# xingbpshen/nested-diffusion

Hardware: AMD Instinct MI355X
Metric: denoising-steps*images/sec (K=5,T=100,224^2) (higher is better)
Workload: dtype f32

## Files before the change

nested_diffusion_amd/csrc/nd_sampler.hip:

```cpp
#include "nd_common.hpp"
#include "nd_step.hpp"
#include "nd_cond_gemm.hpp"
#include "nd_b9.hpp"
#include "nd_persist.hpp"
#include "nd_rng.hpp"
#include "../../include/nested_diffusion.h"

#include <map>
#include <string>
#include <tuple>
#include <vector>
#include <cstdio>
#include <cstdarg>
#include <cstring>
#include <cstdlib>

static thread_local std::string g_err;
extern "C" const char* nd_last_error(void) { return g_err.c_str(); }
#ifdef ND_WG_TIMING
int nd_debug_set_wg_times_m0(void*); int nd_debug_set_wg_times_m1(void*); int nd_debug_set_wg_times_m2(void*);
extern "C" int nd_debug_set_wg_times(void* dev_ptr) {
    return (nd_debug_set_wg_times_m0(dev_ptr) | nd_debug_set_wg_times_m1(dev_ptr) | nd_debug_set_wg_times_m2(dev_ptr)) ? -1 : 0;
}
#endif
// ... 87 lines not shown
            zz[c] = ND_GC(io.noise)[z * io.noise_ms + ((size_t)i_step * M + m) * C + c];
        }
    }
    if (mode == ND_HEAD_UPDATE) {
        al = ND_GC(io.alphas)[t_prev]; s_t = ND_GC(io.omabs)[t_prev]; s_tm1 = ND_GC(io.omabs)[t_prev - 1];
#pragma unroll
        for (int c = 0; c < C; ++c) yo[c] = yold[c];
        nd_reduce_eps<256, C>(mb.epart, NT, m, red, eps);
    }
#pragma unroll
    for (int c = 0; c < C; ++c) {
        if (mode == ND_HEAD_INIT) yv[c] = zz[c] + ym[c];
        else if (mode == ND_HEAD_UPDATE) yv[c] = nd_posterior(yo[c], ym[c], eps[c] + ND_GC(mb.lin4_b)[c], zz[c], al, s_t, s_tm1);
        else yv[c] = ND_GC(io.y_in)[z * io.yin_ms + (size_t)m * C + c];
        if (tid == 0 && blockIdx.x == 0) {
            ynew[c] = yv[c];
            if (io.seq_out && mode != ND_HEAD_GIVEN) ND_GW(io.seq_out)[z * io.seq_ms + ((size_t)i_step * M + m) * C + c] = yv[c];
        }
    }
    if (!live) return;
    float4 h;
    h.x = nd_head_element<C>(w1[0], yv, yh, a.x, cc.x, xe.x);
    h.y = nd_head_element<C>(w1[1], yv, yh, a.y, cc.y, xe.y);
    h.z = nd_head_element<C>(w1[2], yv, yh, a.z, cc.z, xe.z);
    h.w = nd_head_element<C>(w1[3], yv, yh, a.w, cc.w, xe.w);
    if (mb.h16 == 2)
        nd_b9_store4(reinterpret_cast<bf16x8*>(mb.h1), F >> 5, m, n, h.x, h.y, h.z, h.w);
    else if (mb.h16)
        *(__attribute__((address_space(1))) f16x4*)(reinterpret_cast<_Float16*>(mb.h1) + nd_pkh(m, n, F >> 5)) =
            f16x4{(_Float16)h.x, (_Float16)h.y, (_Float16)h.z, (_Float16)h.w};
    else
        *(__attribute__((address_space(1))) f32x4*)(mb.h1 + nd_pk(m, n, nchF)) = f32x4{h.x, h.y, h.z, h.w};
}

#ifndef ND_HEAD_ROWS_COLS
#define ND_HEAD_ROWS_COLS 512
#endif
template <int C>
__global__ __launch_bounds__(256) void k_step_head_rows(MemberInline mi, const MemberDev* __restrict__ members, StepIO io, int mode,
                                                        int i_step, int t_prev, int t, int B, int M, int maxM, int F, int NT, int T) {
    typedef const __attribute__((address_space(4))) char* nd_cbytes;
    const MemberDev mb = nd_ldc<MemberDev>((members ? (nd_cbytes)(uintptr_t)members : (nd_cbytes)__builtin_amdgcn_kernarg_segment_ptr()) +
                                           (size_t)blockIdx.z * sizeof(MemberDev));
    const int z = blockIdx.z, tid = threadIdx.x, m0 = blockIdx.y * 16;
    constexpr int C2 = 2 * C;
    __shared__ float ys[16][C], yhs[16][C];
    {
        const int r = tid >> 4, j = tid & 15, m = min(m0 + r, M - 1), b = m % B;
        const int par_new = i_step & 1;
        nd_gf ynew = ND_GW(mb.ybuf + ((size_t)par_new * maxM + m) * C);
        nd_gcf yold = ND_GC(mb.ybuf + ((size_t)(par_new ^ 1) * maxM + m) * C);
        float yv[C], yh[C], ym[C], zz[C], yo[C], eps[C];
        float al = 0.f, s_t = 0.f, s_tm1 = 0.f;
#pragma unroll
        for (int c = 0; c < C; ++c) {
            yh[c] = ND_GC(io.yhat)[z * io.yhat_ms + (size_t)b * C + c];
            eps[c] = 0.f; ym[c] = 0.f; zz[c] = 0.f; yo[c] = 0.f;
        }
        if (mode != ND_HEAD_GIVEN) {
#pragma unroll
            for (int c = 0; c < C; ++c) {
                ym[c] = ND_GC(io.ymean)[z * io.ymean_ms + (size_t)b * C + c];
                zz[c] = ND_GC(io.noise)[z * io.noise_ms + ((size_t)i_step * M + m) * C + c];
            }
        }
        if (mode == ND_HEAD_UPDATE) {
            al = ND_GC(io.alphas)[t_prev]; s_t = ND_GC(io.omabs)[t_prev]; s_tm1 = ND_GC(io.omabs)[t_prev - 1];
#pragma unroll
            for (int c = 0; c < C; ++c) {
                yo[c] = yold[c];
                nd_gcf row = ND_GC(mb.epart + ((size_t)m * C + c) * NT);
                float q[4];
#pragma unroll
                for (int k = 0; k < 4; ++k) {
                    const int tl = j + 16 * k;
                    const float v = row[min(tl, NT - 1)];
                    q[k] = tl < NT ? 0.f + v : 0.f;
                }
                float s = (q[0] + q[2]) + (q[1] + q[3]);
#pragma unroll
                for (int off = 8; off > 0; off >>= 1) s += __shfl_down(s, off, 16);
                float tot = 0.f;
                tot += s;
                tot += 0.f; tot += 0.f; tot += 0.f;
                eps[c] = __shfl(tot, 0, 16);
            }
        }
#pragma unroll
        for (int c = 0; c < C; ++c) {
            if (mode == ND_HEAD_INIT) yv[c] = zz[c] + ym[c];
            else if (mode == ND_HEAD_UPDATE) yv[c] = nd_posterior(yo[c], ym[c], eps[c] + ND_GC(mb.lin4_b)[c], zz[c], al, s_t, s_tm1);
            else yv[c] = ND_GC(io.y_in)[z * io.yin_ms + (size_t)m * C + c];
            if (j == 0) {
                ys[r][c] = yv[c]; yhs[r][c] = yh[c];
                if (blockIdx.x == 0 && m0 + r < M) {
                    ynew[c] = yv[c];
                    if (io.seq_out && mode != ND_HEAD_GIVEN) ND_GW(io.seq_out)[z * io.seq_ms + ((size_t)i_step * M + m) * C + c] = yv[c];
                }
            }
        }
    }
    __syncthreads();
    const int lane = tid & 63, wave = tid >> 6, r = lane & 15, kq = lane >> 4;
    const int m = m0 + r, b = min(m, M - 1) % B, nkb = F >> 5, nchF = F >> 4;
    float yv[C], yh[C];
#pragma unroll
    for (int c = 0; c < C; ++c) { yv[c] = ys[r][c]; yh[c] = yhs[r][c]; }
    bf16x8* img = reinterpret_cast<bf16x8*>(mb.h1);
#pragma unroll
    for (int it = 0; it < ND_HEAD_ROWS_COLS / 128; ++it) {
        const int kb = blockIdx.x * (ND_HEAD_ROWS_COLS / 32) + wave * (ND_HEAD_ROWS_COLS / 128) + it;
        if (kb >= nkb) break;
        const int n = kb * 32 + kq * 8;
        const float4 a0 = nd_ld16<false>(mb.A1 + (size_t)t * F + n), a1 = nd_ld16<false>(mb.A1 + (size_t)t * F + n + 4);
        const float4 c0 = nd_ld16<false>(mb.C1 + (size_t)t * F + n), c1 = nd_ld16<false>(mb.C1 + (size_t)t * F + n + 4);
        const float4 x0 = nd_ld16<false>(mb.xe + nd_pk(b, n, nchF)), x1 = nd_ld16<false>(mb.xe + nd_pk(b, n + 4, nchF));
        const float av[8] = {a0.x, a0.y, a0.z, a0.w, a1.x, a1.y, a1.z, a1.w};
        const float cv[8] = {c0.x, c0.y, c0.z, c0.w, c1.x, c1.y, c1.z, c1.w};
        const float xv[8] = {x0.x, x0.y, x0.z, x0.w, x1.x, x1.y, x1.z, x1.w};
        nd_gcf wrow = ND_GC(mb.lin1_w + (size_t)n * C2);
        float w1[8][C2];
#pragma unroll
        for (int jj = 0; jj < 8; ++jj)
#pragma unroll
            for (int q = 0; q < C2; ++q) w1[jj][q] = wrow[jj * C2 + q];
        bf16x8 p1, p2, p3;
#pragma unroll
        for (int jj = 0; jj < 8; ++jj) {
            const float hv = nd_head_element<C>(w1[jj], yv, yh, av[jj], cv[jj], xv[jj]);
            __bf16 e1, e2, e3;
            nd_b9_split(hv, e1, e2, e3);
            p1[jj] = e1; p2[jj] = e2; p3[jj] = e3;
        }
        if (m < M) {
            __attribute__((address_space(1))) bf16x8* q = (__attribute__((address_space(1))) bf16x8*)(img + ((size_t)(m0 >> 4) * nkb + kb) * B9_BLOCK_UNITS + lane);
            q[0] = p1; q[64] = p2; q[128] = p3;
        }
    }
}

static void* head_rows_fn(int C) {
    switch (C) {
        case 1: return (void*)k_step_head_rows<1>;
        case 2: return (void*)k_step_head_rows<2>;
        case 3: return (void*)k_step_head_rows<3>;
        case 4: return (void*)k_step_head_rows<4>;
        case 5: return (void*)k_step_head_rows<5>;
        case 6: return (void*)k_step_head_rows<6>;
        case 7: return (void*)k_step_head_rows<7>;
        default: return (void*)k_step_head_rows<8>;
    }
}

static void* head_fn(int C) {
    switch (C) {
        case 1: return (void*)k_step_head<1>;
        case 2: return (void*)k_step_head<2>;
        case 3: return (void*)k_step_head<3>;
        case 4: return (void*)k_step_head<4>;
        case 5: return (void*)k_step_head<5>;
        case 6: return (void*)k_step_head<6>;
        case 7: return (void*)k_step_head<7>;
        default: return (void*)k_step_head<8>;
    }
}

template <int C>
__global__ __launch_bounds__(64) void k_step_final(MemberInline mi, const MemberDev* __restrict__ members, StepIO io, int eps_only, int par_cur,
                                                   int B, int M, int maxM, int NT, int T, float* eps_out, size_t eps_ms) {
    typedef const __attribute__((address_space(4))) char* nd_cbytes;
    const MemberDev mb = nd_ldc<MemberDev>((members ? (nd_cbytes)(uintptr_t)members : (nd_cbytes)__builtin_amdgcn_kernarg_segment_ptr()) +
                                           (size_t)blockIdx.z * sizeof(MemberDev));
    const int z = blockIdx.z, m = blockIdx.x, b = m % B;
    __shared__ float red[C];
    float epsv[C];
    nd_reduce_eps<64, C>(mb.epart, NT, m, red, epsv);
#pragma unroll
    for (int c = 0; c < C; ++c) {
        const float eps = epsv[c] + mb.lin4_b[c];
        if (threadIdx.x == 0) {
            if (eps_only == 1) {
                eps_out[z * eps_ms + (size_t)m * C + c] = eps;
            } else if (eps_only >= 2) {
                const float y = io.y_in[(size_t)m * C + c];
                const float ymean = io.ymean[(size_t)b * C + c];
                const int t = par_cur;
                eps_out[(size_t)m * C + c] = eps_only == 2
                    ? nd_posterior(y, ymean, eps, io.noise[(size_t)m * C + c], io.alphas[t], io.omabs[t], io.omabs[t - 1])
                    : nd_y0_reparam(y, ymean, eps, io.omabs[0]);
            } else {
                const float y = mb.ybuf[((size_t)par_cur * maxM + m) * C + c];
                const float ymean = io.ymean[z * io.ymean_ms + (size_t)b * C + c];
                const float y0 = nd_y0_reparam(y, ymean, eps, io.omabs[0]);
                io.y0_out[z * io.y0_ms + (size_t)m * C + c] = y0;
                if (io.seq_out) io.seq_out[z * io.seq_ms + ((size_t)T * M + m) * C + c] = y0;
            }
        }
    }
}

static void* final_fn(int C) {
    switch (C) {
        case 1: return (void*)k_step_final<1>;
        case 2: return (void*)k_step_final<2>;
        case 3: return (void*)k_step_final<3>;
        case 4: return (void*)k_step_final<4>;
        case 5: return (void*)k_step_final<5>;
        case 6: return (void*)k_step_final<6>;
        case 7: return (void*)k_step_final<7>;
        default: return (void*)k_step_final<8>;
    }
}

__global__ void k_fold_bn(float* scale, float* shift, const float* lin_b, const float* bn_w, const float* bn_b,
                          const float* bn_mean, const float* bn_var, int N) {
    const int n = blockIdx.x * blockDim.x + threadIdx.x;
    if (n >= N) return;
    const double s = (double)bn_w[n] / sqrt((double)bn_var[n] + 1e-5);
    const double o = (double)bn_b[n] - (double)bn_mean[n] * s;
    scale[n] = (float)s;
    shift[n] = (float)(s * (double)lin_b[n] + o);
}
__global__ void k_fold_steps(float* A, float* Cc, const float* emb, const float* lin_b, const float* bn_w, const float* bn_b,
                             const float* bn_mean, const float* bn_var, int T, int N) {
    const size_t i = (size_t)blockIdx.x * blockDim.x + threadIdx.x;
    if (i >= (size_t)T * N) return;
    const int n = (int)(i % N);
    const double s = (double)bn_w[n] / sqrt((double)bn_var[n] + 1e-5);
    const double o = (double)bn_b[n] - (double)bn_mean[n] * s;
    const double g = (double)emb[i];
    A[i] = (float)(s * g);
    Cc[i] = (float)(s * g * (double)lin_b[n] + o);
}

#define ND_KEEP_BYTES 208.0e6
enum { L_ENC0 = 0, L_ENC1 = 1, L_ENC2 = 2, L_LIN2 = 3, L_LIN3 = 4, L_LIN2S = 5, L_LIN3S = 6, L_COUNT = 7 };

struct MemberHost {
    bool loaded = false;
    float *sc0, *sh0, *sc1, *sh1, *sc2, *sh2;
    float *A[3], *Cc[3];
    float *w_enc0, *w_enc3, *w_enc6, *w_lin2, *w_lin3;
    float *w_lin1, *w_lin4, *b_lin4;
    float *e0, *e1, *xe, *ybuf, *h1, *h2, *epart, *splitk;
    void *w_lin2s = nullptr, *w_lin3s = nullptr, *h1s = nullptr, *h2s = nullptr;
    bool h_split = false;
};

struct GraphKey {
    int m0, nm, B, mc, T;
    const void *yhat, *ymean, *noise, *y0, *seq;
    bool operator<(const GraphKey& o) const {
        return std::tie(m0, nm, B, mc, T, yhat, ymean, noise, y0, seq) <
               std::tie(o.m0, o.nm, o.B, o.mc, o.T, o.yhat, o.ymean, o.noise, o.y0, o.seq);
    }
};

int nd_guiding_prediction_first(nd_cond c, const float* images, float* logits_out, float* yhat_out, int B, int n_used, void* stream);
unsigned long long nd_cond_serial(nd_cond c);

struct BatchKey {
    unsigned long long cond;
    const void *images, *noise, *samples, *prob, *vote, *probs, *yhat;
    int B, mc, T;
    unsigned temp_bits;
    bool profiling;
    bool operator<(const BatchKey& o) const {
        return std::tie(cond, images, noise, samples, prob, vote, probs, yhat, B, mc, T, temp_bits, profiling) <
               std::tie(o.cond, o.images, o.noise, o.samples, o.prob, o.vote, o.probs, o.yhat, o.B, o.mc, o.T, o.temp_bits, o.profiling);
    }
};

struct nd_handle_s {
    nd_config cfg{};
    char* ws = nullptr;
    size_t ws_bytes = 0;
    std::vector<MemberHost> members;
    MemberDev* members_dev = nullptr;
    SkinnyDesc* descs_dev = nullptr;
    std::vector<SkinnyDesc> descs_host;
    std::vector<MemberDev> members_host;
    SkinnyDesc* spk_dev = nullptr;
    SplitKEpiDesc* spke_dev = nullptr;
    float *alphas = nullptr, *omabs = nullptr;
    float* xpack = nullptr;
    float* tile_ws = nullptr;
    bool b9 = false;
    unsigned long long* rng_state = nullptr;
    unsigned* input_seq = nullptr;
    unsigned* input_flag = nullptr;
    unsigned* persist_bar = nullptr;
    int persist_mode = 0;
    int persist_skew_ticks = 0;
    bool persist_last = false;
    float* noise_ws = nullptr;
    float* logits_ws = nullptr;
    int sched_T = 0;
    int NT = 0, S0 = 0;
    bool enc_splitk = false;
    int half = 0;
    std::map<GraphKey, hipGraphExec_t> graphs;
    std::map<BatchKey, hipGraphExec_t> batch_graphs;
    hipStream_t capture_stream = nullptr;
    int encoded_B = -1;
    bool profiling = false;
    std::vector<hipEvent_t> probe_events;
    int probe_steps = 0;
    int probe_nodes = 0;
};

static inline size_t al256(size_t x) { return (x + 255) & ~(size_t)255; }

struct Carver {
    char* base; size_t off = 0;
    template <typename T> T* take(size_t count) {
        T* p = base ? reinterpret_cast<T*>(base + off) : nullptr;
        off = al256(off + count * sizeof(T));
// ... 283 lines not shown
    return encode_impl(h, m0, nm, x_dev, B, stream, false);
}

static int encode_impl(nd_handle h, int m0, int nm, const float* x_dev, int B, void* stream, bool signal_inputs) {
    int rc = check_range(h, m0, nm);
    if (rc != ND_OK) return rc;
    if (!x_dev) return nd_set_err(ND_ERR_ARG, "x_dev is NULL");
    if (B < 1 || B > h->cfg.max_batch) return nd_set_err(ND_ERR_ARG, "B=%d outside [1,%d]", B, h->cfg.max_batch);
    hipStream_t st = (hipStream_t)stream;
    const nd_config& c = h->cfg;
    const int K = c.n_members, H = c.hidden_dim, F = c.feature_dim, D = c.data_dim;
    launch_pack(x_dev, h->xpack, B, D, h->half, st);
    if (signal_inputs && h->input_flag)
        hipLaunchKernelGGL(k_inputs_consumed, dim3(1), dim3(1), 0, st, h->input_seq, h->input_flag);
    if (h->enc_splitk) {
        const SkinnyLaunch L = nd_skinny_launch<2>(D, H, B, nm, h->half);
        HIP_CHECK(nd_launch_skinny(L, SkinnyDesc{}, h->spk_dev + m0, nm, B, 0, st));
        const size_t q = (size_t)(((B + 15) / 16) * 16) * H / 4;
        hipLaunchKernelGGL(k_splitk_epilogue, dim3((unsigned)((q + 255) / 256), 1, nm), dim3(256), 0, st, SplitKEpiDesc{},
                           (const SplitKEpiDesc*)(h->spke_dev + m0), B, L.S);
    } else {
        HIP_CHECK(launch_skinny<0>(h->descs_dev + (size_t)L_ENC0 * K + m0, D, H, B, 0, nm, h->half, st));
    }
    HIP_CHECK(launch_skinny<0>(h->descs_dev + (size_t)L_ENC1 * K + m0, H, H, B, 0, nm, h->half, st));
    HIP_CHECK(launch_skinny<0>(h->descs_dev + (size_t)L_ENC2 * K + m0, H, F, B, 0, nm, h->half, st));
    HIP_CHECK(hipGetLastError());
    h->encoded_B = B;
    return ND_OK;
}

extern "C" int nd_member_buffer(nd_handle h, int k, int which, float* dst_dev, int rows, void* stream) {
    if (!h || !dst_dev) return nd_set_err(ND_ERR_ARG, "bad argument");
    if (k < 0 || k >= h->cfg.n_members) return nd_set_err(ND_ERR_ARG, "member out of range");
    if (which < 0 || which > 4) return nd_set_err(ND_ERR_ARG, "which=%d unknown", which);
    if (rows < 1 || rows > h->cfg.max_rows) return nd_set_err(ND_ERR_ARG, "rows out of range");
    const bool enc = which == 0 || which >= 3;
    if (enc && rows > h->cfg.max_batch) return nd_set_err(ND_ERR_ARG, "%s holds at most max_batch rows", which == 0 ? "xe" : which == 3 ? "e0" : "e1");
    if (!h->ws) return nd_set_err(ND_ERR_STATE, "workspace not bound");
    MemberHost& m = h->members[k];
    const float* src = which == 0 ? m.xe : which == 1 ? m.h1 : which == 2 ? m.h2 : which == 3 ? m.e0 : m.e1;
    const int W = which >= 3 ? h->cfg.hidden_dim : h->cfg.feature_dim;
    if (!enc && m.h_split) return nd_join_rows(which == 1 ? m.h1s : m.h2s, dst_dev, rows, W, stream);
    const size_t n4 = (size_t)((rows + 15) / 16) * 16 * W / 4;
    if (h->half && which != 0)
        hipLaunchKernelGGL(k_unpack_rows_h, dim3((unsigned)((n4 / 2 + 255) / 256)), dim3(256), 0, (hipStream_t)stream,
                           reinterpret_cast<const _Float16*>(src), dst_dev, rows, W);
    else
        hipLaunchKernelGGL(k_unpack_rows, dim3((unsigned)((n4 + 255) / 256)), dim3(256), 0, (hipStream_t)stream, src, dst_dev, rows, W);
    HIP_CHECK(hipGetLastError());
    return ND_OK;
}

extern "C" long long nd_resident_weight_bytes(nd_handle h, int block) {
    if (!h || block < 0 || block > 1 || h->descs_host.empty()) return -1;
    const int K = h->cfg.n_members, F = h->cfg.feature_dim;
    long long n = 0;
    for (int k = 0; k < K; ++k)
        if (h->members[k].loaded && h->descs_host[(size_t)(block ? L_LIN3 : L_LIN2) * K + k].keep) n += (long long)F * F * (h->half ? 2 : 4);
    return n;
}

extern "C" int nd_set_profiling(nd_handle h, int enable) {
    if (!h) return nd_set_err(ND_ERR_ARG, "handle is NULL");
    if (h->profiling != (enable != 0)) drop_graphs(h);
    h->profiling = enable != 0;
    return ND_OK;
}

extern "C" int nd_set_loop_form(nd_handle h, int mode, float skew_us) {
    if (!h) return nd_set_err(ND_ERR_ARG, "handle is NULL");
    if (mode != 0 && mode != 1) return nd_set_err(ND_ERR_ARG, "mode must be 0 (per-step kernels) or 1 (one launch per loop)");
    if (skew_us > 1e6f) return nd_set_err(ND_ERR_ARG, "skew_us out of range");
    h->persist_mode = mode;
    if (skew_us >= 0.f) h->persist_skew_ticks = (int)(skew_us * 100.0f);
    drop_graphs(h);
    return ND_OK;
}

extern "C" int nd_loop_form(nd_handle h) { return h && h->persist_last ? 1 : 0; }

extern "C" int nd_persist_status(nd_handle h, int reset) {
    if (!h || !h->ws) return nd_set_err(ND_ERR_STATE, "workspace not bound");
    HIP_CHECK(hipDeviceSynchronize());
    unsigned flag = 0;
    HIP_CHECK(hipMemcpy(&flag, h->persist_bar + ND_PERSIST_ERR_WORD, sizeof flag, hipMemcpyDeviceToHost));
    if (reset && flag) HIP_CHECK(hipMemset(h->persist_bar, 0, ND_PERSIST_BAR_WORDS * sizeof(unsigned)));
    return flag ? 1 : 0;
}

static int count_event_record_nodes(hipGraph_t g) {
    size_t n = 0;
    if (hipGraphGetNodes(g, nullptr, &n) != hipSuccess) return -1;
    std::vector<hipGraphNode_t> nodes(n);
    if (n && hipGraphGetNodes(g, nodes.data(), &n) != hipSuccess) return -1;
    int cnt = 0;
    for (size_t i = 0; i < n; ++i) {
        hipGraphNodeType ty;
        if (hipGraphNodeGetType(nodes[i], &ty) != hipSuccess) return -1;
        if (ty == hipGraphNodeTypeEventRecord) ++cnt;
    }
    return cnt;
}

extern "C" int nd_profile_probe_nodes(nd_handle h) {
    if (!h) return nd_set_err(ND_ERR_ARG, "handle is NULL");
    return h->probe_nodes;
}

extern "C" int nd_profile_read(nd_handle h, float* out_us, int* n_samples) {
    if (!h || !out_us || !n_samples) return nd_set_err(ND_ERR_ARG, "NULL argument");
    double acc[3] = {0, 0, 0};
    const int n = h->probe_steps;
    for (int s = 0; s < n; ++s)
        for (int k = 0; k < 3; ++k) {
            float ms = 0.f;
            HIP_CHECK(hipEventElapsedTime(&ms, h->probe_events[4 * s + k], h->probe_events[4 * s + k + 1]));
            acc[k] += ms * 1000.0;
        }
    out_us[0] = n ? (float)(acc[0] / n) : 0.f;
    out_us[1] = n ? (float)(acc[1] / n) : 0.f;
    out_us[2] = n ? (float)(acc[2] / n) : 0.f;
    const float head = out_us[2] - out_us[1];
    out_us[3] = n ? (out_us[0] - head > 0.f ? out_us[0] - head : 0.f) : 0.f;
    *n_samples = n;
    return ND_OK;
}

static int check_rows(nd_handle_s* h, int B, int mc, int T) {
    if (B < 1 || B > h->cfg.max_batch) return nd_set_err(ND_ERR_ARG, "B=%d outside [1,%d]", B, h->cfg.max_batch);
    if (mc < 1 || mc > 65535 || (long)B * mc > h->cfg.max_rows)
        return nd_set_err(ND_ERR_ARG, "mc=%d outside [1,65535] or B*mc=%ld exceeds max_rows=%d", mc, (long)B * mc, h->cfg.max_rows);
    if (T < 1 || T > h->cfg.n_steps) return nd_set_err(ND_ERR_ARG, "T=%d outside [1,%d]", T, h->cfg.n_steps);
    if (h->sched_T < T) return nd_set_err(ND_ERR_STATE, "schedule holds %d steps, need %d (nd_set_schedule)", h->sched_T, T);
    if (h->encoded_B != B) return nd_set_err(ND_ERR_STATE, "nd_encode ran with B=%d, sampling asks B=%d", h->encoded_B, B);
    return ND_OK;
}

static bool loop_writes_split(const nd_handle_s* h, int M, int nm) {
    return h->b9 && nm <= ND_INLINE_DESCS && nd_cond_gemm_plan(h->cfg.feature_dim, h->cfg.feature_dim, M, nm, h->half).use_tile;
}
static void note_h_layout(nd_handle_s* h, int m0, int nm, bool split) {
    for (int k = m0; k < m0 + nm; ++k) h->members[k].h_split = split;
}

static int single_eval(nd_handle_s* h, int member, StepIO io, int t, int final_mode, float* out, int B, int mc, hipStream_t st) {
    const nd_config& c = h->cfg;
    const int K = c.n_members, F = c.feature_dim, C = c.y_dim, M = B * mc;
    note_h_layout(h, member, 1, false);
    {
        const MemberDev* mdev = h->members_dev + member;
        MemberInline mi{};
        int mode = ND_HEAD_GIVEN, istep = 0, tprev = 0, tt = t, Bv = B, Mv = M, maxM = c.max_rows, Fv = F, NT = step_partials(h, M), Tn = c.n_steps;
        void* ah[] = {&mi, &mdev, &io, &mode, &istep, &tprev, &tt, &Bv, &Mv, &maxM, &Fv, &NT, &Tn};
        HIP_CHECK(hipLaunchKernel(head_fn(C), dim3((F + 1023) / 1024, M, 1), dim3(256), ah, 0, st));
    }
    HIP_CHECK(launch_step_block<0>(h, h->descs_dev + (size_t)L_LIN2 * K + member, M, t, 1, st));
    HIP_CHECK(launch_step_block<1>(h, h->descs_dev + (size_t)L_LIN3 * K + member, M, t, 1, st));
    {
        const MemberDev* mdev = h->members_dev + member;
        MemberInline mi{};
        int fm = final_mode, tt = t, Bv = B, Mv = M, maxM = c.max_rows, NT = step_partials(h, M), Tn = c.n_steps;
        size_t ems = 0;
        void* af[] = {&mi, &mdev, &io, &fm, &tt, &Bv, &Mv, &maxM, &NT, &Tn, &out, &ems};
        HIP_CHECK(hipLaunchKernel(final_fn(C), dim3(M, 1, 1), dim3(64), af, 0, st));
    }
    HIP_CHECK(hipGetLastError());
    return ND_OK;
}

extern "C" int nd_eps_theta(nd_handle h, int member, const float* y_dev, const float* yhat_dev, int t, float* eps_out, int B,
                            int mc, void* stream) {
    int rc = check_range(h, member, 1);
    if (rc != ND_OK) return rc;
    if (!y_dev || !yhat_dev || !eps_out) return nd_set_err(ND_ERR_ARG, "NULL tensor");
    if (B < 1 || B > h->cfg.max_batch || mc < 1 || (long)B * mc > h->cfg.max_rows) return nd_set_err(ND_ERR_ARG, "B/mc out of range");
    if (t < 0 || t >= h->cfg.n_steps) return nd_set_err(ND_ERR_ARG, "t=%d outside [0,%d)", t, h->cfg.n_steps);
    if (h->encoded_B != B) return nd_set_err(ND_ERR_STATE, "nd_encode ran with B=%d, asked B=%d", h->encoded_B, B);
    StepIO io{};
    io.yhat = yhat_dev; io.y_in = y_dev; io.alphas = h->alphas; io.omabs = h->omabs;
    return single_eval(h, member, io, t, 1, eps_out, B, mc, (hipStream_t)stream);
}

extern "C" int nd_p_sample(nd_handle h, int member, const float* y_dev, const float* yhat_dev, const float* ymean_dev,
                           const float* z_dev, int t, float* y_out, int B, int mc, void* stream) {
    int rc = check_range(h, member, 1);
    if (rc != ND_OK) return rc;
    if (!y_dev || !yhat_dev || !ymean_dev || !y_out) return nd_set_err(ND_ERR_ARG, "NULL tensor");
    if (t < 0) return nd_set_err(ND_ERR_ARG, "t must be >= 0");
    if (t > 0 && !z_dev) return nd_set_err(ND_ERR_ARG, "z_dev is required for t >= 1");
    rc = check_rows(h, B, mc, t + 1);
    if (rc != ND_OK) return rc;
    StepIO io{};
    io.yhat = yhat_dev; io.ymean = ymean_dev; io.y_in = y_dev; io.noise = z_dev; io.alphas = h->alphas; io.omabs = h->omabs;
    return single_eval(h, member, io, t, t > 0 ? 2 : 3, y_out, B, mc, (hipStream_t)stream);
}

struct Emitter {
    hipStream_t st;
    hipGraph_t graph = nullptr;
    hipGraphNode_t last = nullptr;
    hipError_t err = hipSuccess;
    bool capturing = false;
    void record(hipEvent_t ev) {
        if (err != hipSuccess) return;
        if (!graph && capturing) {
            hipStreamCaptureStatus cs = hipStreamCaptureStatusNone;
            unsigned long long id = 0;
            hipGraph_t g = nullptr;
            const hipGraphNode_t* deps = nullptr;
            size_t ndeps = 0;
            err = hipStreamGetCaptureInfo_v2(st, &cs, &id, &g, &deps, &ndeps);
            if (err != hipSuccess) return;
            if (cs != hipStreamCaptureStatusActive || !g) { err = hipErrorStreamCaptureInvalidated; return; }
            hipGraphNode_t node;
            err = hipGraphAddEventRecordNode(&node, g, deps, ndeps, ev);
            if (err != hipSuccess) return;
            err = hipStreamUpdateCaptureDependencies(st, &node, 1, hipStreamSetCaptureDependencies);
        } else if (!graph) {
            err = hipEventRecord(ev, st);
        } else {
            hipGraphNode_t node;
            err = hipGraphAddEventRecordNode(&node, graph, last ? &last : nullptr, last ? 1 : 0, ev);
            last = node;
        }
    }
    void emit(void* fn, dim3 grid, dim3 block, void** args, size_t lds = 0) {
        if (err != hipSuccess) return;
        if (!graph) {
            err = hipLaunchKernel(fn, grid, block, args, lds, st);
        } else {
            hipKernelNodeParams p{};
            p.func = fn; p.gridDim = grid; p.blockDim = block; p.sharedMemBytes = (unsigned)lds; p.kernelParams = args; p.extra = nullptr;
            hipGraphNode_t node;
            err = hipGraphAddKernelNode(&node, graph, last ? &last : nullptr, last ? 1 : 0, &p);
            last = node;
        }
    }
};

static hipError_t emit_loop(nd_handle_s* h, Emitter& em, int m0, int nm, StepIO io, int B, int mc, int T) {
    const nd_config& c = h->cfg;
    int K = c.n_members, F = c.feature_dim, C = c.y_dim, M = B * mc, maxM = c.max_rows, NT = step_partials(h, M), Tn = T;
    const bool inl = nm <= ND_INLINE_DESCS;
    const MemberDev* mdev = inl ? nullptr : h->members_dev + m0;
    const SkinnyDesc* t2 = h->descs_dev + (size_t)L_LIN2 * K + m0;
    const SkinnyDesc* t3 = h->descs_dev + (size_t)L_LIN3 * K + m0;
    const SkinnyDesc *s2 = inl ? nullptr : t2, *s3 = inl ? nullptr : t3;
    MemberInline mi{};
    SkinnyInline i2{}, i3{};
    for (int g = 0; inl && g < nm; ++g) {
        mi.m[g] = h->members_host[m0 + g];
        i2.d[g] = h->descs_host[(size_t)L_LIN2 * K + m0 + g];
        i3.d[g] = h->descs_host[(size_t)L_LIN3 * K + m0 + g];
    }
    h->persist_last = false;
    if (h->persist_mode && inl) {
        const PersistPlan pp = nd_persist_plan(F, M, nm, C, h->half);
        if (pp.ok) {
            if (pp.err != hipSuccess) return pp.err;
            PersistArgs pa{};
            for (int g = 0; g < nm; ++g) { pa.l2[g] = i2.d[g]; pa.l3[g] = i3.d[g]; pa.mem[g] = mi.m[g]; }
            pa.io = io;
            const char* act = getenv("ND_PERSIST_ACTIVE");
            const char* spin = getenv("ND_PERSIST_SPIN_TICKS");
            const char* fake = getenv("ND_PERSIST_FAKE_RESIDENT");
            pa.s = PersistScalars{h->persist_bar, nm, B, M, maxM, F, T, h->persist_skew_ticks, spin ? atoi(spin) : 100000000 ,
                                  act ? atoi(act) : nm, fake ? atoi(fake) : 0};
            note_h_layout(h, m0, nm, false);
            hipEvent_t* ev = nullptr;
            if (h->profiling) {
                if (h->probe_events.size() < 4) {
                    const size_t old = h->probe_events.size();
                    h->probe_events.resize(4);
                    for (size_t e = old; e < 4; ++e)
                        if (hipEventCreate(&h->probe_events[e]) != hipSuccess) return hipErrorOutOfMemory;
                }
                ev = h->probe_events.data();
            }
            if (ev) em.record(ev[0]);
            void* ap[] = {&pa};
            em.emit(pp.fn, pp.grid, pp.block, ap, pp.lds);
            if (ev) em.record(ev[1]);
            h->probe_steps = 0;
            h->persist_last = true;
            return em.err;
        }
    }
    SkinnyDesc d0{};
    const dim3 ghead((F + 1023) / 1024, M, nm);
    const SkinnyLaunch L2 = nd_skinny_launch<0>(F, F, M, nm, h->half), L3 = nd_skinny_launch<1>(F, F, M, nm, h->half);
    if (L2.err != hipSuccess) return L2.err;
    if (L3.err != hipSuccess) return L3.err;
    int cps2 = L2.cps, cps3 = L3.cps;
    CondGemmPlan tp = nd_cond_gemm_plan(F, F, M, nm, h->half);
    float* tws = h->tile_ws;
    const bool b9 = tp.use_tile && h->b9 && inl;
    note_h_layout(h, m0, nm, b9);
    if (b9) {
        t2 = h->descs_dev + (size_t)L_LIN2S * K + m0;
        t3 = h->descs_dev + (size_t)L_LIN3S * K + m0;
        for (int g = 0; g < nm; ++g) { mi.m[g].h1 = (float*)h->members[m0 + g].h1s; mi.m[g].h16 = 2; }
    }
    const dim3 tgrid((unsigned)(tp.n_full + tp.rem * tp.split)), tfix((unsigned)tp.rem * (b9 ? 16 : 4));
    const bool rows_head = b9 && NT <= 64 && !getenv("ND_HEAD_PER_ROW");
    const dim3 ghead_rows((F + ND_HEAD_ROWS_COLS - 1) / ND_HEAD_ROWS_COLS, (M + 15) / 16, nm);
    const int want = h->profiling ? ((T - 1) / 2 < 8 ? (T - 1) / 2 : 8) : 0;
    const int stride = want > 0 ? (T - 1) / want : 0;
    hipEvent_t pending_end = nullptr;
    if ((int)h->probe_events.size() < 4 * want) {
        const size_t old = h->probe_events.size();
        h->probe_events.resize(4 * want);
        for (size_t e = old; e < h->probe_events.size(); ++e)
            if (hipEventCreate(&h->probe_events[e]) != hipSuccess) return hipErrorOutOfMemory;
    }
    int probed = 0;
    for (int i = 0; i < T; ++i) {
        int t = T - 1 - i, t_prev = t + 1, mode = (i == 0) ? ND_HEAD_INIT : ND_HEAD_UPDATE, istep = i;
        const bool probe = want > 0 && i >= 1 && i + 1 < T && !pending_end && probed < want && ((i - 1) % stride) == (stride - 1) / 2;
        hipEvent_t* ev = probe ? &h->probe_events[4 * probed] : nullptr;
        hipEvent_t end_of_pair = pending_end;
        pending_end = nullptr;
        if (probe) em.record(ev[0]);
        void* ah[] = {&mi, &mdev, &io, &mode, &istep, &t_prev, &t, &B, &M, &maxM, &F, &NT, &Tn};
        em.emit(rows_head ? head_rows_fn(C) : head_fn(C), rows_head ? ghead_rows : ghead, dim3(256), ah);
        if (probe) em.record(ev[1]);
        if (tp.use_tile) {
            void* a2[] = {&d0, &t2, &M, &t, &tp.TM, &tp.TN, &tp.n_full, &tp.split, &tws};
            void* a3[] = {&d0, &t3, &M, &t, &tp.TM, &tp.TN, &tp.n_full, &tp.split, &tws};
            if (b9) {
                em.emit(nd_cond_gemm_b9_kernel(0), tgrid, dim3(512), a2, nd_cond_gemm_b9_dynlds());
                if (tp.rem > 0) em.emit(nd_cond_gemm_b9_fixup_kernel(0), tfix, dim3(64), a2);
                em.emit(nd_cond_gemm_b9_kernel(1), tgrid, dim3(512), a3, nd_cond_gemm_b9_dynlds());
                if (tp.rem > 0) em.emit(nd_cond_gemm_b9_fixup_kernel(1), tfix, dim3(64), a3);
            } else {
                em.emit(nd_cond_gemm_kernel(0), tgrid, dim3(256), a2, nd_cond_gemm_dynlds());
                if (tp.rem > 0) em.emit(nd_cond_gemm_fixup_kernel(0), tfix, dim3(64), a2);
                em.emit(nd_cond_gemm_kernel(1), tgrid, dim3(256), a3, nd_cond_gemm_dynlds());
                if (tp.rem > 0) em.emit(nd_cond_gemm_fixup_kernel(1), tfix, dim3(64), a3);
            }
        } else {
            void* a2[] = {&i2, &s2, &nm, &M, &t, &cps2};
            em.emit(L2.fn, L2.grid, L2.block, a2, L2.lds);
            void* a3[] = {&i3, &s3, &nm, &M, &t, &cps3};
            em.emit(L3.fn, L3.grid, L3.block, a3, L3.lds);
        }
        if (probe) { em.record(ev[2]); pending_end = ev[3]; ++probed; }
        if (end_of_pair) em.record(end_of_pair);
    }
    h->probe_steps = probed;
    int eps_only = 0, par_cur = (T - 1) & 1;
    float* eps_out = nullptr;
    size_t eps_ms = 0;
    void* af[] = {&mi, &mdev, &io, &eps_only, &par_cur, &B, &M, &maxM, &NT, &Tn, &eps_out, &eps_ms};
    em.emit(final_fn(C), dim3(M, 1, nm), dim3(64), af);
    return em.err;
}

static int run_loop_eager(nd_handle_s* h, hipStream_t st, int m0, int nm, StepIO io, bool draw, int B, int mc, int T) {
    if (draw) HIP_CHECK(nd_launch_philox_normal(h->noise_ws, h->rng_state, 0, 0, 0, m0, nm, T, B, mc, h->cfg.y_dim, st));
    Emitter em{st};
    hipStreamCaptureStatus cs = hipStreamCaptureStatusNone;
    HIP_CHECK(hipStreamIsCapturing(st, &cs));
    em.capturing = cs == hipStreamCaptureStatusActive;
    hipError_t e = emit_loop(h, em, m0, nm, io, B, mc, T);
    if (e != hipSuccess) return nd_set_err(ND_ERR_HIP, "kernel launch failed: %s", hipGetErrorString(e));
    if (draw) HIP_CHECK(nd_launch_rng_advance(h->rng_state, st));
    return ND_OK;
}

extern "C" int nd_sample(nd_handle h, int m0, int nm, const float* yhat_dev, const float* ymean_dev, const float* noise_dev,
                         float* y0_out_dev, float* seq_out_dev, int B, int mc, int T, int use_graph, void* stream) {
    int rc = check_range(h, m0, nm);
    if (rc != ND_OK) return rc;
    if (!yhat_dev || !ymean_dev || !y0_out_dev) return nd_set_err(ND_ERR_ARG, "NULL tensor");
    rc = check_rows(h, B, mc, T);
    if (rc != ND_OK) return rc;
    hipStream_t st = (hipStream_t)stream;
    const int C = h->cfg.y_dim, M = B * mc;
    const bool draw = noise_dev == nullptr;
    StepIO io{};
    io.yhat = yhat_dev;   io.yhat_ms = (size_t)B * C;
    io.ymean = ymean_dev; io.ymean_ms = (size_t)B * C;
    io.noise = draw ? h->noise_ws : noise_dev; io.noise_ms = (size_t)T * M * C;
    io.y0_out = y0_out_dev; io.y0_ms = (size_t)M * C;
    io.seq_out = seq_out_dev; io.seq_ms = (size_t)(T + 1) * M * C;
    io.alphas = h->alphas; io.omabs = h->omabs;
    if (!use_graph) return run_loop_eager(h, st, m0, nm, io, draw, B, mc, T);
    GraphKey key{m0, nm, B, mc, T, yhat_dev, ymean_dev, noise_dev, y0_out_dev, seq_out_dev};
    auto it = h->graphs.find(key);
    if (it == h->graphs.end()) {
        Emitter em{st};
        HIP_CHECK(hipGraphCreate(&em.graph, 0));
        if (draw) {
            float* out = h->noise_ws;
            const unsigned long long* state = h->rng_state;
            unsigned long long seed0 = 0;
            uint32_t z0 = 0, z1 = 0;
            int m0v = m0, nmv = nm, Tv = T, Bv = B, mcv = mc, Cv = C;
            void* a[] = {&out, &state, &seed0, &z0, &z1, &m0v, &nmv, &Tv, &Bv, &mcv, &Cv};
            const size_t total = (size_t)nm * T * M * ((C + 3) / 4);
            em.emit(nd_philox_normal_kernel(), dim3((unsigned)((total + 255) / 256)), dim3(256), a);
        }
        hipError_t e = emit_loop(h, em, m0, nm, io, B, mc, T);
        if (e == hipSuccess && draw) {
            unsigned long long* state = h->rng_state;
            void* a[] = {&state};
            em.emit(nd_rng_advance_kernel(), dim3(1), dim3(64), a);
            e = em.err;
        }
        if (e != hipSuccess) {
            (void)hipGraphDestroy(em.graph);
            return nd_set_err(ND_ERR_HIP, "graph build failed: %s", hipGetErrorString(e));
        }
        h->probe_nodes = count_event_record_nodes(em.graph);
        hipGraphExec_t exec;
        e = hipGraphInstantiate(&exec, em.graph, nullptr, nullptr, 0);
        (void)hipGraphDestroy(em.graph);
        if (e != hipSuccess) return nd_set_err(ND_ERR_HIP, "hipGraphInstantiate failed: %s", hipGetErrorString(e));
        if (h->graphs.size() >= 64) drop_graphs(h);
        it = h->graphs.emplace(key, exec).first;
    }
    HIP_CHECK(hipGraphLaunch(it->second, st));
    note_h_layout(h, m0, nm, loop_writes_split(h, M, nm));
    return ND_OK;
}

static int batch_enqueue(nd_handle_s* h, nd_cond c, const float* images, const float* noise, const nd_batch_out* out, int B, int mc,
                         int T, float temperature, hipStream_t st) {
    const int K = h->cfg.n_members, C = h->cfg.y_dim, M = B * mc;
    const bool draw = noise == nullptr;
    int rc = nd_guiding_prediction_first(c, images, h->logits_ws, out->yhat, B, K, st);
    if (rc != ND_OK) return rc;
    rc = encode_impl(h, 0, K, images, B, st, true);
    if (rc != ND_OK) return rc;
    StepIO io{};
    io.yhat = out->yhat;  io.yhat_ms = (size_t)B * C;
    io.ymean = out->yhat; io.ymean_ms = (size_t)B * C;
    io.noise = draw ? h->noise_ws : noise; io.noise_ms = (size_t)T * M * C;
    io.y0_out = out->samples; io.y0_ms = (size_t)M * C;
    io.alphas = h->alphas; io.omabs = h->omabs;
    rc = run_loop_eager(h, st, 0, K, io, draw, B, mc, T);
    if (rc != ND_OK) return rc;
    return nd_aggregate(out->samples, out->prob, out->vote, out->probs, K * mc, B, C, temperature, st);
}

extern "C" int nd_predict_batch(nd_handle h, nd_cond c, const float* images_dev, const float* noise_dev, const nd_batch_out* out,
                                int B, int mc, int T, float temperature, int use_graph, void* stream) {
    if (!h || !h->ws) return nd_set_err(ND_ERR_STATE, "workspace not bound");
    if (!c) return nd_set_err(ND_ERR_ARG, "conditioner is NULL");
    if (!images_dev || !out || !out->samples || !out->prob || !out->vote || !out->yhat) return nd_set_err(ND_ERR_ARG, "NULL tensor");
    const nd_cond_config* cc = nd_cond_get_config(c);
    const nd_config& g = h->cfg;
    if (cc->n_mlps < g.n_members) return nd_set_err(ND_ERR_ARG, "conditioner has %d mapping MLPs, ensemble %d members", cc->n_mlps, g.n_members);
    if (cc->num_classes != g.y_dim) return nd_set_err(ND_ERR_ARG, "conditioner has %d classes, ensemble %d", cc->num_classes, g.y_dim);
    if ((long)cc->in_chans * cc->img_size * cc->img_size != g.data_dim)
        return nd_set_err(ND_ERR_ARG, "image size %dx%dx%d != data_dim %d", cc->in_chans, cc->img_size, cc->img_size, g.data_dim);
    int rc = check_range(h, 0, g.n_members);
    if (rc != ND_OK) return rc;
    if (B < 1 || B > g.max_batch || B > cc->max_batch) return nd_set_err(ND_ERR_ARG, "B=%d outside [1,%d]", B, g.max_batch < cc->max_batch ? g.max_batch : cc->max_batch);
    if (mc < 1 || mc > 65535 || (long)B * mc > g.max_rows)
        return nd_set_err(ND_ERR_ARG, "mc=%d outside [1,65535] or B*mc=%ld exceeds max_rows=%d", mc, (long)B * mc, g.max_rows);
    if (T < 1 || T > g.n_steps) return nd_set_err(ND_ERR_ARG, "T=%d outside [1,%d]", T, g.n_steps);
    if (h->sched_T < T) return nd_set_err(ND_ERR_STATE, "schedule holds %d steps, need %d (nd_set_schedule)", h->sched_T, T);
    if (!(temperature > 0.f)) return nd_set_err(ND_ERR_ARG, "temperature must be > 0");
    hipStream_t st = (hipStream_t)stream;
    if (!use_graph) return batch_enqueue(h, c, images_dev, noise_dev, out, B, mc, T, temperature, st);
    unsigned tb;
    memcpy(&tb, &temperature, sizeof tb);
    BatchKey key{nd_cond_serial(c), images_dev, noise_dev, out->samples, out->prob, out->vote, out->probs, out->yhat, B, mc, T, tb, h->profiling};
    auto it = h->batch_graphs.find(key);
    if (it == h->batch_graphs.end()) {
        rc = batch_enqueue(h, c, images_dev, noise_dev, out, B, mc, T, temperature, st);
        if (rc != ND_OK) return rc;
        if (!h->capture_stream) HIP_CHECK(hipStreamCreateWithFlags(&h->capture_stream, hipStreamNonBlocking));
        HIP_CHECK(hipStreamBeginCapture(h->capture_stream, hipStreamCaptureModeRelaxed));
        rc = batch_enqueue(h, c, images_dev, noise_dev, out, B, mc, T, temperature, h->capture_stream);
        hipGraph_t graph = nullptr;
// ... 22 lines not shown
```

Baseline: 783,300.

## Add fragment-layout head kernel for non-tiled streaming GEMM path

Adds a new head kernel that computes the first-layer activations and writes them directly in a 16-row fragment layout (fp16 or fp32) for the streaming lin2/lin3 block kernels. It prefetches operands for the next block of features in registers to overlap loads with compute. The kernel is used whenever the tiled conditional GEMM plan is not selected, for both the sampler loop and single evaluation. The aim is to improve how the head's output feeds the following GEMM, at the cost of a new kernel variant that depends on the downstream kernels expecting this exact fragment layout.

After: 766,700. -2.1%, worse.

```diff
diff --git a/nested_diffusion_amd/csrc/nd_sampler.hip b/nested_diffusion_amd/csrc/nd_sampler.hip
--- a/nested_diffusion_amd/csrc/nd_sampler.hip
+++ b/nested_diffusion_amd/csrc/nd_sampler.hip
@@ -263,6 +263,146 @@
     }
 }
 
+#ifndef ND_HEAD_FRAG_BLOCKS
+#define ND_HEAD_FRAG_BLOCKS 2
+#endif
+template <int C, int H>
+__global__ __launch_bounds__(256) void k_step_head_frag(MemberInline mi, const MemberDev* __restrict__ members, StepIO io, int mode,
+                                                        int i_step, int t_prev, int t, int B, int M, int maxM, int F, int NT, int T) {
+    typedef const __attribute__((address_space(4))) char* nd_cbytes;
+    const MemberDev mb = nd_ldc<MemberDev>((members ? (nd_cbytes)(uintptr_t)members : (nd_cbytes)__builtin_amdgcn_kernarg_segment_ptr()) +
+                                           (size_t)blockIdx.z * sizeof(MemberDev));
+    const int z = blockIdx.z, tid = threadIdx.x, m0 = blockIdx.y * 16;
+    constexpr int C2 = 2 * C, V = H ? 2 : 1;
+    const int lane = tid & 63, wave = tid >> 6, lr = lane & 15, kq = lane >> 4;
+    const int nblk = F / (16 * V), nchF = F >> 4;
+    const int ml = m0 + lr, bl = min(ml, M - 1) % B;
+    const int blk0 = blockIdx.x * (4 * ND_HEAD_FRAG_BLOCKS) + wave;
+    struct Operands { float4 a[V], cc[V], xe[V]; float w1[4 * V][C2]; };
+    auto load = [&](int blk) {
+        Operands o;
+        const int n = blk * (16 * V) + kq * (4 * V);
+#pragma unroll
+        for (int v = 0; v < V; ++v) {
+            o.a[v] = nd_ld16<false>(mb.A1 + (size_t)t * F + n + 4 * v);
+            o.cc[v] = nd_ld16<false>(mb.C1 + (size_t)t * F + n + 4 * v);
+            o.xe[v] = nd_ld16<false>(mb.xe + nd_pk(bl, n + 4 * v, nchF));
+        }
+        nd_gcf wrow = ND_GC(mb.lin1_w + (size_t)n * C2);
+#pragma unroll
+        for (int jj = 0; jj < 4 * V; ++jj)
+#pragma unroll
+            for (int q = 0; q < C2; ++q) o.w1[jj][q] = wrow[jj * C2 + q];
+        return o;
+    };
+    Operands nxt = load(min(blk0, nblk - 1));
+    __shared__ float ys[16][C], yhs[16][C];
+    {
+        const int r = tid >> 4, j = tid & 15, m = min(m0 + r, M - 1), b = m % B;
+        const int par_new = i_step & 1;
+        nd_gf ynew = ND_GW(mb.ybuf + ((size_t)par_new * maxM + m) * C);
+        nd_gcf yold = ND_GC(mb.ybuf + ((size_t)(par_new ^ 1) * maxM + m) * C);
+        float yv[C], yh[C], ym[C], zz[C], yo[C], eps[C];
+        float al = 0.f, s_t = 0.f, s_tm1 = 0.f;
+#pragma unroll
+        for (int c = 0; c < C; ++c) {
+            yh[c] = ND_GC(io.yhat)[z * io.yhat_ms + (size_t)b * C + c];
+            eps[c] = 0.f; ym[c] = 0.f; zz[c] = 0.f; yo[c] = 0.f;
+        }
+        if (mode != ND_HEAD_GIVEN) {
+#pragma unroll
+            for (int c = 0; c < C; ++c) {
+                ym[c] = ND_GC(io.ymean)[z * io.ymean_ms + (size_t)b * C + c];
+                zz[c] = ND_GC(io.noise)[z * io.noise_ms + ((size_t)i_step * M + m) * C + c];
+            }
+        }
+        if (mode == ND_HEAD_UPDATE) {
+            al = ND_GC(io.alphas)[t_prev]; s_t = ND_GC(io.omabs)[t_prev]; s_tm1 = ND_GC(io.omabs)[t_prev - 1];
+#pragma unroll
+            for (int c = 0; c < C; ++c) {
+                yo[c] = yold[c];
+                nd_gcf row = ND_GC(mb.epart + ((size_t)m * C + c) * NT);
+                float tot = 0.f;
+#pragma unroll
+                for (int w = 0; w < 4; ++w) {
+                    float q[4];
+#pragma unroll
+                    for (int k = 0; k < 4; ++k) {
+                        const int tl = 64 * w + 16 * k + j;
+                        const float v = row[min(tl, NT - 1)];
+                        float s = tl < NT ? 0.f + v : 0.f;
+                        for (int tl2 = tl + 256; tl2 < NT; tl2 += 256) s += row[tl2];
+                        q[k] = s;
+                    }
+                    float s = (q[0] + q[2]) + (q[1] + q[3]);
+#pragma unroll
+                    for (int off = 8; off > 0; off >>= 1) s += __shfl_down(s, off, 16);
+                    tot += s;
+                }
+                eps[c] = __shfl(tot, 0, 16);
+            }
+        }
+#pragma unroll
+        for (int c = 0; c < C; ++c) {
+            if (mode == ND_HEAD_INIT) yv[c] = zz[c] + ym[c];
+            else if (mode == ND_HEAD_UPDATE) yv[c] = nd_posterior(yo[c], ym[c], eps[c] + ND_GC(mb.lin4_b)[c], zz[c], al, s_t, s_tm1);
+            else yv[c] = ND_GC(io.y_in)[z * io.yin_ms + (size_t)m * C + c];
+            if (j == 0) {
+                ys[r][c] = yv[c]; yhs[r][c] = yh[c];
+                if (blockIdx.x == 0 && m0 + r < M) {
+                    ynew[c] = yv[c];
+                    if (io.seq_out && mode != ND_HEAD_GIVEN) ND_GW(io.seq_out)[z * io.seq_ms + ((size_t)i_step * M + m) * C + c] = yv[c];
+                }
+            }
+        }
+    }
+    __syncthreads();
+    float yv[C], yh[C];
+#pragma unroll
+    for (int c = 0; c < C; ++c) { yv[c] = ys[lr][c]; yh[c] = yhs[lr][c]; }
+#pragma unroll
+    for (int it = 0; it < ND_HEAD_FRAG_BLOCKS; ++it) {
+        const int blk = blk0 + 4 * it;
+        if (blk >= nblk) break;
+        const Operands o = nxt;
+        if (it + 1 < ND_HEAD_FRAG_BLOCKS) nxt = load(min(blk + 4, nblk - 1));
+        float hv[4 * V];
+#pragma unroll
+        for (int v = 0; v < V; ++v) {
+            hv[4 * v + 0] = nd_head_element<C>(o.w1[4 * v + 0], yv, yh, o.a[v].x, o.cc[v].x, o.xe[v].x);
+            hv[4 * v + 1] = nd_head_element<C>(o.w1[4 * v + 1], yv, yh, o.a[v].y, o.cc[v].y, o.xe[v].y);
+            hv[4 * v + 2] = nd_head_element<C>(o.w1[4 * v + 2], yv, yh, o.a[v].z, o.cc[v].z, o.xe[v].z);
+            hv[4 * v + 3] = nd_head_element<C>(o.w1[4 * v + 3], yv, yh, o.a[v].w, o.cc[v].w, o.xe[v].w);
+        }
+        if (ml >= M)
+#pragma unroll
+            for (int e = 0; e < 4 * V; ++e) hv[e] = 0.f;
+        const size_t unit = ((size_t)(m0 >> 4) * nblk + blk) * 64 + lane;
+        if (H) {
+            f16x8 p;
+#pragma unroll
+            for (int e = 0; e < 8; ++e) p[e] = (_Float16)hv[e];
+            ((__attribute__((address_space(1))) f16x8*)mb.h1)[unit] = p;
+        } else {
+            ((__attribute__((address_space(1))) f32x4*)mb.h1)[unit] = f32x4{hv[0], hv[1], hv[2], hv[3]};
+        }
+    }
+}
+
+template <int H>
+static void* head_frag_fn(int C) {
+    switch (C) {
+        case 1: return (void*)k_step_head_frag<1, H>;
+        case 2: return (void*)k_step_head_frag<2, H>;
+        case 3: return (void*)k_step_head_frag<3, H>;
+        case 4: return (void*)k_step_head_frag<4, H>;
+        case 5: return (void*)k_step_head_frag<5, H>;
+        case 6: return (void*)k_step_head_frag<6, H>;
+        case 7: return (void*)k_step_head_frag<7, H>;
+        default: return (void*)k_step_head_frag<8, H>;
+    }
+}
+
 static void* head_fn(int C) {
     switch (C) {
         case 1: return (void*)k_step_head<1>;
@@ -274,6 +414,12 @@
         case 7: return (void*)k_step_head<7>;
         default: return (void*)k_step_head<8>;
     }
+}
+
+static void* stream_head_fn(int C, int half) { return half ? head_frag_fn<1>(C) : head_frag_fn<0>(C); }
+static dim3 stream_head_grid(int F, int M, int nm, int half) {
+    const int nblk = F / (half ? 32 : 16), per_wg = 4 * ND_HEAD_FRAG_BLOCKS;
+    return dim3((nblk + per_wg - 1) / per_wg, (M + 15) / 16, nm);
 }
 
 template <int C>
@@ -863,7 +1009,9 @@
         MemberInline mi{};
         int mode = ND_HEAD_GIVEN, istep = 0, tprev = 0, tt = t, Bv = B, Mv = M, maxM = c.max_rows, Fv = F, NT = step_partials(h, M), Tn = c.n_steps;
         void* ah[] = {&mi, &mdev, &io, &mode, &istep, &tprev, &tt, &Bv, &Mv, &maxM, &Fv, &NT, &Tn};
-        HIP_CHECK(hipLaunchKernel(head_fn(C), dim3((F + 1023) / 1024, M, 1), dim3(256), ah, 0, st));
+        const bool stream_blocks = !nd_cond_gemm_plan(F, F, M, 1, h->half).use_tile;
+        if (stream_blocks) HIP_CHECK(hipLaunchKernel(stream_head_fn(C, h->half), stream_head_grid(F, M, 1, h->half), dim3(256), ah, 0, st));
+        else HIP_CHECK(hipLaunchKernel(head_fn(C), dim3((F + 1023) / 1024, M, 1), dim3(256), ah, 0, st));
     }
     HIP_CHECK(launch_step_block<0>(h, h->descs_dev + (size_t)L_LIN2 * K + member, M, t, 1, st));
     HIP_CHECK(launch_step_block<1>(h, h->descs_dev + (size_t)L_LIN3 * K + member, M, t, 1, st));
@@ -1033,7 +1181,8 @@
         pending_end = nullptr;
         if (probe) em.record(ev[0]);
         void* ah[] = {&mi, &mdev, &io, &mode, &istep, &t_prev, &t, &B, &M, &maxM, &F, &NT, &Tn};
-        em.emit(rows_head ? head_rows_fn(C) : head_fn(C), rows_head ? ghead_rows : ghead, dim3(256), ah);
+        if (!tp.use_tile) em.emit(stream_head_fn(C, h->half), stream_head_grid(F, M, nm, h->half), dim3(256), ah);
+        else em.emit(rows_head ? head_rows_fn(C) : head_fn(C), rows_head ? ghead_rows : ghead, dim3(256), ah);
         if (probe) em.record(ev[1]);
         if (tp.use_tile) {
             void* a2[] = {&d0, &t2, &M, &t, &tp.TM, &tp.TN, &tp.n_full, &tp.split, &tws};
```
